# mwickert/scikit-dsp-comm

Measured on AMD Instinct MI355X. Metric: complex64 MSamples/s (FIR-1024 tap, 2^26 samples), higher is better.
Workload: dtype c64

## Files before the change

### scikit-dsp-comm_amd/csrc/fir_ols.hip

```cpp
#include "skdsp_internal.hpp"
#include "ols_tables.hpp"
#include "fir_route.hpp"
#include <cstdlib>
#include <cstdio>


namespace skdsp {

using namespace ols;
typedef float v4f_t __attribute__((ext_vector_type(4)));

struct OlsPlan : TilePlan {
    int ntaps = 0;
    int ov = 0;
    int V = 0;
    DevTable<float4> T1, T2, Hp;
};

struct OlsArgs {
    const cf *x;
    cf *y;
    int64_t n, n_hist;
    const float4 *T1, *T2, *Hp;
    int ov, V, a0;
    int keep;
    int aligned;
    int64_t ntiles;
    int dec;
    unsigned dec_magic;
    int up;
    int64_t up_pitch;
    int up_sb, up_pbs, up_pb0;
    int64_t n_keep;
    const unsigned *halo_flag;
    unsigned halo_seq;
    unsigned *halo_err;
    int halo_spins;
    CarefulFir cf;
    int rep_L, rep_lr;
    unsigned rep_magic;
    int64_t n_in, rep_hist;
};

__device__ __forceinline__ void wait_halo(const OlsArgs &A)
{
    if (threadIdx.x == 0) {
        int spins = 0;
        while ((int)(__hip_atomic_load(A.halo_flag, __ATOMIC_RELAXED, __HIP_MEMORY_SCOPE_AGENT) - A.halo_seq) < 0) {
            if (++spins > A.halo_spins) {
                *A.halo_err = 1u;
                break;
            }
            __builtin_amdgcn_s_sleep(16);
        }
        __builtin_amdgcn_fence(__ATOMIC_ACQUIRE, "agent");
    }
    __syncthreads();
}

static inline int ols_keep_blocks(int a0)
{
    const int o = opt().ols_keep_overlap;
    return o == 0 ? 0 : (o == 1 ? a0 : 8);
}

__device__ __forceinline__ float4 vld(const volatile float4 *p)
{
    float4 r;
    r.x = p->x; r.y = p->y; r.z = p->z; r.w = p->w;
    return r;
}

#define SK_GLOBAL_PTR(T, p) ((__attribute__((address_space(1))) T *)(p))
struct ScalarBase {
    uint64_t b;
    int g = 0;
    __device__ __forceinline__ explicit ScalarBase(const void *start) : b(reinterpret_cast<uint64_t>(start)) { asm volatile("" : "+s"(b)); }
    template <class T> __device__ __forceinline__ __attribute__((address_space(1))) T *at(int d, unsigned off)
    {
        const int gn = (d + 4096) >> 13;
        if (gn != g) {
            b += (uint64_t)(int64_t)(8192 * (gn - g));
            asm volatile("" : "+s"(b));
            g = gn;
        }
        return reinterpret_cast<__attribute__((address_space(1))) T *>(SK_GLOBAL_PTR(char, b) + off + (d - 8192 * gn));
    }
};

template <int KEEP, int A> __device__ __forceinline__ void load_tile_block(ScalarBase &xb, unsigned off, cf *v)
{
    const __attribute__((address_space(1))) v4f_t *src = xb.at<const v4f_t>(A * 4096, off);
    v4f_t nv;
    if constexpr (A < KEEP || A >= 16 - KEEP) nv = *src;
    else nv = __builtin_nontemporal_load(src);
    const float4 f = make_float4(nv.x, nv.y, nv.z, nv.w);
    v[2 * A] = lo(f);
    v[2 * A + 1] = hi(f);
    if constexpr (A < 15) load_tile_block<KEEP, A + 1>(xb, off, v);
}
template <int KEEP> __device__ __forceinline__ void load_tile_blocks(const cf *x0, int t, cf *v)
{
    int tt = t;
    asm volatile("" : "+v"(tt));
    ScalarBase xb(x0);
    load_tile_block<KEEP, 0>(xb, 16u * (unsigned)tt, v);
}

__device__ __forceinline__ void load_tile(const OlsArgs &A, int64_t tile, int t, cf *v)
{
    const int64_t in0 = tile * A.V - A.ov;
    const bool interior = A.aligned && in0 >= -A.n_hist && in0 + kN <= A.n;
    if (interior) {
        switch (A.keep) {
            case 0: load_tile_blocks<0>(A.x + in0, t, v); break;
            case 1: load_tile_blocks<1>(A.x + in0, t, v); break;
            case 2: load_tile_blocks<2>(A.x + in0, t, v); break;
            case 3: load_tile_blocks<3>(A.x + in0, t, v); break;
            case 4: load_tile_blocks<4>(A.x + in0, t, v); break;
            case 5: load_tile_blocks<5>(A.x + in0, t, v); break;
            case 6: load_tile_blocks<6>(A.x + in0, t, v); break;
            case 7: load_tile_blocks<7>(A.x + in0, t, v); break;
            default: load_tile_blocks<8>(A.x + in0, t, v); break;
        }
// ... 311 lines not shown
    const int64_t left = A.n - outA;
    const int lim = (left > (1 << 20) ? (1 << 20) : (int)left) - pos;
    const int limb = lim - A.V;
    const bool whole = left >= 2 * (int64_t)A.V;
    const unsigned b0 = (unsigned)pos * (unsigned)A.up_sb, b1 = b0 + 64u * (unsigned)A.up_sb;
    const size_t step = (size_t)512 * A.up_sb;
    const unsigned M = (unsigned)A.dec;
    const int64_t jt = outA * A.up + ph, q0 = DEC ? jt / A.dec : 0;
    const unsigned r0 = DEC ? (unsigned)(jt - q0 * A.dec) : 0u;
    const int64_t qleft = A.n_keep - q0;
    const int qlim = qleft > (1 << 24) ? (1 << 24) : (int)qleft;
    float *yq = reinterpret_cast<float *>(A.y) + q0;
    const unsigned jv = (unsigned)A.V * (unsigned)A.up;
#pragma unroll
    for (int a = 0; a < 16; ++a) {
        if (a < a0) continue;
        cf e0 = v[2 * a], e1 = v[2 * a + 1];
        lanes_swap_halves(e0.x, e1.x);
        lanes_swap_halves(e0.y, e1.y);
        const int i = 512 * (a - a0);
        if (DEC) {
            const unsigned j0 = r0 + (unsigned)(i + pos) * (unsigned)A.up, j1 = j0 + 64u * (unsigned)A.up;
            auto keep = [&](unsigned j, float val, bool inside) __attribute__((always_inline)) {
                const unsigned k = (unsigned)(((unsigned long long)j * A.dec_magic) >> 32);
                if (k * M == j && (int)k < qlim && inside) yq[k] = val;
            };
            keep(j0, e0.x, whole || i < lim);
            keep(j1, e1.x, whole || i + 64 < lim);
            keep(j0 + jv, e0.y, whole || i < limb);
            keep(j1 + jv, e1.y, whole || i + 64 < limb);
            continue;
        }
        char *ua = ua0 + (size_t)(a - a0) * step, *ub = ub0 + (size_t)(a - a0) * step;
        if (whole || i < lim) *reinterpret_cast<float *>(ua + b0) = e0.x;
        if (whole || i + 64 < lim) *reinterpret_cast<float *>(ua + b1) = e1.x;
        if (whole || i < limb) *reinterpret_cast<float *>(ub + b0) = e0.y;
        if (whole || i + 64 < limb) *reinterpret_cast<float *>(ub + b1) = e1.y;
    }
}


__device__ __forceinline__ OlsCareful ols_careful_args(const OlsArgs &A, int ph, bool cx)
{
    OlsCareful c;
    c.x = A.x; c.y = A.y; c.n = A.n; c.n_hist = A.n_hist; c.n_keep = A.n_keep; c.up_pitch = A.up_pitch;
    c.V = A.V; c.dec = A.dec; c.up = A.up;
    const int esz = cx ? 8 : 4;
    c.L = A.up_sb / esz;
    c.p0 = (A.up_pb0 + ph * A.up_pbs) / esz;
    c.cf = A.cf;
    return c;
}

template <bool REAL, bool DEC, bool UP = false, bool XR = false>
__global__ __launch_bounds__(256, 2) void ols_tile_kernel(OlsArgs A)
{
    __shared__ float4 lds[kLdsUnits];
    __shared__ float4 t2lds[2 * kT2Units];
    __shared__ unsigned long long ols_noted;
    if (threadIdx.x == 0) ols_noted = 0;
    constexpr int HS = (DEC && !UP) ? (REAL ? 4 : 5) : 0;
    float4 *T2f = t2lds;
    float4 *T2t = t2lds + kT2Units;
    const int t = threadIdx.x;

    {
        const float4 w = A.T2[t];
        T2f[t] = w;
        T2t[(t & 15) * 16 + (t >> 4)] = w;
    }
    cf tw[16];
#pragma unroll
    for (int k1 = 1; k1 < 16; ++k1) tw[k1] = lo(A.T1[k1 * 256 + t]);
    tw[0] = make_float2(1.f, 0.f);

    __syncthreads();
    int it = 0;
    float4 hh[16];
    int64_t tile = (gridDim.x % 8 == 0) ? (int64_t)(blockIdx.x % 8) * (gridDim.x / 8) + blockIdx.x / 8
                                                                 : (int64_t)blockIdx.x;
    const bool t0_last = A.halo_flag != nullptr;
    auto phys = [&](int64_t w) -> int64_t {
        if (UP) return (int64_t)__builtin_amdgcn_readfirstlane((unsigned)w / (unsigned)A.up);
        return t0_last ? (w + 1 < A.ntiles ? w + 1 : 0) : w;
    };
    auto phase_of = [&](int64_t w) -> int { return (int)__builtin_amdgcn_readfirstlane((unsigned)w % (unsigned)A.up); };
    if (!UP) load_H(t, A.Hp, hh);
    cf v[32];
    if (tile < A.ntiles) {
        if (t0_last && phys(tile) == 0) wait_halo(A);
        load_any<REAL, XR>(A, phys(tile), t, v);
    }
    if constexpr (XR) {
#pragma unroll
        for (int i = 0; i < 32; i += 8)
            asm volatile("" ::"v"(v[i].x), "v"(v[i + 1].x), "v"(v[i + 2].x), "v"(v[i + 3].x), "v"(v[i + 4].x), "v"(v[i + 5].x), "v"(v[i + 6].x), "v"(v[i + 7].x));
    } else {
#pragma unroll
    for (int i = 0; i < 32; i += 8)
        asm volatile("" ::"v"(v[i].x), "v"(v[i].y), "v"(v[i + 1].x), "v"(v[i + 1].y), "v"(v[i + 2].x), "v"(v[i + 2].y),
                     "v"(v[i + 3].x), "v"(v[i + 3].y), "v"(v[i + 4].x), "v"(v[i + 4].y), "v"(v[i + 5].x), "v"(v[i + 5].y),
                     "v"(v[i + 6].x), "v"(v[i + 6].y), "v"(v[i + 7].x), "v"(v[i + 7].y));
    }
    for (; tile < A.ntiles; tile += gridDim.x, ++it) {
        if (HS > 0) {
            int tt = t;
            asm volatile("" : "+v"(tt));
#pragma unroll
            for (int j = 16 - HS; j < 16; ++j) hh[j] = vld(reinterpret_cast<const volatile float4 *>(A.Hp) + (unsigned)(j * 256 + tt));
        }
        if (UP) {
            int tt = t;
            asm volatile("" : "+v"(tt));
            const volatile float4 *hp = reinterpret_cast<const volatile float4 *>(A.Hp) + (size_t)phase_of(tile) * 4096;
#pragma unroll
            for (int j = 0; j < 16; ++j) hh[j] = vld(hp + (unsigned)(j * 256 + tt));
        }
        if (REAL) fwd_pass1_real(t, v, tw, lds); else fwd_pass1(t, v, tw, lds);
        __syncthreads();
        cf Z[32];
        fwd_pass23(t, T2f, lds, Z);
        mul_H(hh, Z);
        const int64_t next = tile + gridDim.x;
        cf nx[32];
        __builtin_amdgcn_s_setprio(3);
        if (next < A.ntiles) {
            if (t0_last && phys(next) == 0) wait_halo(A);
            load_any<REAL, XR>(A, phys(next), t, nx);
        }
        __builtin_amdgcn_s_setprio(0);
        inv_pass32(t, T2t, lds, Z);
        __syncthreads();
        inv_pass1(t, tw, lds, v);
        if constexpr (XR) {
#pragma unroll
            for (int i = 0; i < 32; i += 8)
                asm volatile("" ::"v"(nx[i].x), "v"(nx[i + 1].x), "v"(nx[i + 2].x), "v"(nx[i + 3].x), "v"(nx[i + 4].x), "v"(nx[i + 5].x), "v"(nx[i + 6].x), "v"(nx[i + 7].x)
                             : "memory");
        } else {
#pragma unroll
        for (int i = 0; i < 32; i += 8)
            asm volatile("" ::"v"(nx[i].x), "v"(nx[i].y), "v"(nx[i + 1].x), "v"(nx[i + 1].y), "v"(nx[i + 2].x), "v"(nx[i + 2].y),
                         "v"(nx[i + 3].x), "v"(nx[i + 3].y), "v"(nx[i + 4].x), "v"(nx[i + 4].y), "v"(nx[i + 5].x), "v"(nx[i + 5].y),
                         "v"(nx[i + 6].x), "v"(nx[i + 6].y), "v"(nx[i + 7].x), "v"(nx[i + 7].y)
                         : "memory");
        }
        __builtin_amdgcn_s_setprio(3);
        if (UP) {
            if (!DEC && A.up_pitch) {
                OlsArgs B = A;
                B.y = REAL ? reinterpret_cast<cf *>(reinterpret_cast<float *>(A.y) + (int64_t)phase_of(tile) * A.up_pitch) : A.y + (int64_t)phase_of(tile) * A.up_pitch;
                store_any<REAL, false>(B, phys(tile), t, v, lds);
            } else if (REAL) {
                store_tile_real_up<DEC>(A, phys(tile), phase_of(tile), t, v);
            } else {
                store_tile_up<DEC>(A, phys(tile), phase_of(tile), t, v);
            }
        } else {
            store_any<REAL, DEC>(A, phys(tile), t, v, lds);
        }
        __builtin_amdgcn_s_setprio(0);
        if (__builtin_expect(__any(not_finite(v[31].x) | not_finite(v[31].y)), 0)) careful_note(&ols_noted, it);
#pragma unroll
        for (int i = 0; i < 32; ++i) v[i] = nx[i];
#ifdef SK_OLS_KEEP_B3
        __syncthreads();
#else
        if constexpr (REAL || DEC || UP || XR) __syncthreads();
#endif
    }
    const unsigned long long noted = careful_noted(&ols_noted);
    if (__builtin_expect(noted != 0, 0)) {
        int64_t w = (gridDim.x % 8 == 0) ? (int64_t)(blockIdx.x % 8) * (gridDim.x / 8) + blockIdx.x / 8 : (int64_t)blockIdx.x;
        for (int64_t k = 0; w < A.ntiles; w += gridDim.x, ++k)
            if (careful_step_noted(noted, k))
                careful_ols_tile<float, REAL, DEC, UP, XR>(ols_careful_args(A, UP ? phase_of(w) : 0, !(REAL || XR)), phys(w), UP ? phase_of(w) : 0, t);
    }
}


template <bool REAL, int MF>
__global__ __launch_bounds__(256, 2) void ols_fold_kernel(OlsArgs A)
{
    __shared__ float4 lds[kLdsUnits];
    __shared__ float4 t2lds[2 * kT2Units];
    __shared__ unsigned long long ols_noted;
    if (threadIdx.x == 0) ols_noted = 0;
    float4 *T2f = t2lds, *T2t = t2lds + kT2Units;
    const int t = threadIdx.x;
    {
        const float4 w = A.T2[t];
        T2f[t] = w;
        T2t[(t & 15) * 16 + (t >> 4)] = w;
    }
    cf tw[16];
#pragma unroll
    for (int k1 = 1; k1 < 16; ++k1) tw[k1] = lo(A.T1[k1 * 256 + t]);
    tw[0] = make_float2(1.f, 0.f);
    __syncthreads();
    float4 hh[16];
    auto first_tile = [&]() -> int64_t { return (gridDim.x % 8 == 0) ? (int64_t)(blockIdx.x % 8) * (gridDim.x / 8) + blockIdx.x / 8 : (int64_t)blockIdx.x; };
    int64_t tile = first_tile();
    load_H(t, A.Hp, hh);
    cf v[32];
    if (tile < A.ntiles) load_any<REAL, false>(A, tile, t, v);
#pragma unroll
    for (int i = 0; i < 32; i += 8)
        asm volatile("" ::"v"(v[i].x), "v"(v[i].y), "v"(v[i + 1].x), "v"(v[i + 1].y), "v"(v[i + 2].x), "v"(v[i + 2].y),
                     "v"(v[i + 3].x), "v"(v[i + 3].y), "v"(v[i + 4].x), "v"(v[i + 4].y), "v"(v[i + 5].x), "v"(v[i + 5].y),
                     "v"(v[i + 6].x), "v"(v[i + 6].y), "v"(v[i + 7].x), "v"(v[i + 7].y));
    constexpr int LS = MF / 2;
    const int b = t >> 4, q = t & 15;
    const bool active = q % LS == 0;
    const int j0 = (32 / MF) * b + q / LS;
    constexpr int JA = 512 / MF;
    for (int64_t step = 0; tile < A.ntiles; tile += gridDim.x, ++step) {
        if (REAL) fwd_pass1_real(t, v, tw, lds); else fwd_pass1(t, v, tw, lds);
        __syncthreads();
        cf Z[32];
        fwd_pass23(t, T2f, lds, Z);
        mul_H(hh, Z);
        const int64_t next = tile + gridDim.x;
        cf nx[32];
        __builtin_amdgcn_s_setprio(3);
        if (next < A.ntiles) load_any<REAL, false>(A, next, t, nx);
        __builtin_amdgcn_s_setprio(0);
        inv_pass32_fold<MF>(t, T2t, lds, Z);
        __syncthreads();
        cf o[16];
#pragma unroll
        for (int a = 0; a < 16; ++a) o[a] = make_float2(0.f, 0.f);
        inv_pass1_fold<MF>(t, tw, lds, o);
#pragma unroll
        for (int i = 0; i < 32; i += 8)
            asm volatile("" ::"v"(nx[i].x), "v"(nx[i].y), "v"(nx[i + 1].x), "v"(nx[i + 1].y), "v"(nx[i + 2].x), "v"(nx[i + 2].y),
                         "v"(nx[i + 3].x), "v"(nx[i + 3].y), "v"(nx[i + 4].x), "v"(nx[i + 4].y), "v"(nx[i + 5].x), "v"(nx[i + 5].y),
                         "v"(nx[i + 6].x), "v"(nx[i + 6].y), "v"(nx[i + 7].x), "v"(nx[i + 7].y)
                         : "memory");
        __builtin_amdgcn_s_setprio(3);
        if (active) {
            int a0 = A.a0;
            asm volatile("" : "+s"(a0));
            const int Mr = A.dec / MF;
            const int64_t n_out = A.n_keep / A.dec;
            const int VD = A.V / MF;
            const int64_t e0 = (REAL ? 2 * tile : tile) * (int64_t)VD;
            const int64_t q0 = Mr > 1 ? e0 / Mr : e0;
            const unsigned r0 = Mr > 1 ? (unsigned)(e0 - q0 * Mr) : 0u;
            auto put = [&](unsigned el, auto val, auto *yp) __attribute__((always_inline)) {
                if (Mr > 1) {
// ... 65 lines not shown
    int tt = j0;
    asm volatile("" : "+v"(tt));
    if (interior) {
        asm volatile("" : "+v"(tt));
        if (REAL) {
            const float *xr = reinterpret_cast<const float *>(A.x) + e0;
            const unsigned off = 4u * (unsigned)tt;
            ScalarBase xa(xr), xb(xr + VD);
#pragma unroll
            for (int a = 0; a < 16; ++a)
                in[a] = make_float2(__builtin_nontemporal_load(xa.at<const float>(JA * 4 * a, off)), __builtin_nontemporal_load(xb.at<const float>(JA * 4 * a, off)));
        } else {
            const unsigned off = 8u * (unsigned)tt;
            ScalarBase xc(A.x + e0);
#pragma unroll
            for (int a = 0; a < 16; ++a) {
                const v2f_t r = __builtin_nontemporal_load(xc.at<const v2f_t>(JA * 8 * a, off));
                in[a] = make_float2(r.x, r.y);
            }
        }
        return;
    }
#pragma unroll
    for (int a = 0; a < 16; ++a) {
        int64_t ia, ib;
        if (REAL) {
            const float *xr = reinterpret_cast<const float *>(A.x);
            float va = 0.f, vb = 0.f;
            if (fetch((unsigned)(JA * a + tt), ia) && ia >= -A.rep_hist && ia < A.n_in) va = xr[ia];
            if (fetch((unsigned)(JA * a + tt + VD), ib) && ib >= -A.rep_hist && ib < A.n_in) vb = xr[ib];
            in[a] = make_float2(va, vb);
        } else if (fetch((unsigned)(JA * a + tt), ia) && ia >= -A.rep_hist && ia < A.n_in) {
            in[a] = A.x[ia];
        }
    }
}

template <bool REAL, int LF>
__global__ __launch_bounds__(256, 2) void ols_rep_kernel(OlsArgs A)
{
    __shared__ float4 lds[kLdsUnits];
    __shared__ float4 t2lds[2 * kT2Units];
    __shared__ unsigned long long ols_noted;
    if (threadIdx.x == 0) ols_noted = 0;
    float4 *T2f = t2lds, *T2t = t2lds + kT2Units;
    const int t = threadIdx.x;
    {
        const float4 w = A.T2[t];
        T2f[t] = w;
        T2t[(t & 15) * 16 + (t >> 4)] = w;
    }
    cf tw[16];
#pragma unroll
    for (int k1 = 1; k1 < 16; ++k1) tw[k1] = lo(A.T1[k1 * 256 + t]);
    tw[0] = make_float2(1.f, 0.f);
    __syncthreads();
    float4 hh[16];
    auto first_tile = [&]() -> int64_t { return (gridDim.x % 8 == 0) ? (int64_t)(blockIdx.x % 8) * (gridDim.x / 8) + blockIdx.x / 8 : (int64_t)blockIdx.x; };
    int64_t tile = first_tile();
    load_H(t, A.Hp, hh);
    cf in[16];
    if (tile < A.ntiles) load_rep<REAL, LF>(A, tile, t, in);
#pragma unroll
    for (int i = 0; i < 16; i += 8)
        asm volatile("" ::"v"(in[i].x), "v"(in[i].y), "v"(in[i + 1].x), "v"(in[i + 1].y), "v"(in[i + 2].x), "v"(in[i + 2].y),
                     "v"(in[i + 3].x), "v"(in[i + 3].y), "v"(in[i + 4].x), "v"(in[i + 4].y), "v"(in[i + 5].x), "v"(in[i + 5].y),
                     "v"(in[i + 6].x), "v"(in[i + 6].y), "v"(in[i + 7].x), "v"(in[i + 7].y));
    for (int64_t step = 0; tile < A.ntiles; tile += gridDim.x, ++step) {
        fwd_pass1_rep<LF>(t, in, tw, lds);
        __syncthreads();
        cf Z[32];
        fwd_pass23_rep<LF>(t, T2f, lds, Z);
        mul_H(hh, Z);
        const int64_t next = tile + gridDim.x;
        cf nx[16];
        __builtin_amdgcn_s_setprio(3);
        if (next < A.ntiles) load_rep<REAL, LF>(A, next, t, nx);
        __builtin_amdgcn_s_setprio(0);
        inv_pass32(t, T2t, lds, Z);
        __syncthreads();
        cf v[32];
        inv_pass1(t, tw, lds, v);
#pragma unroll
        for (int i = 0; i < 16; i += 8)
            asm volatile("" ::"v"(nx[i].x), "v"(nx[i].y), "v"(nx[i + 1].x), "v"(nx[i + 1].y), "v"(nx[i + 2].x), "v"(nx[i + 2].y),
                         "v"(nx[i + 3].x), "v"(nx[i + 3].y), "v"(nx[i + 4].x), "v"(nx[i + 4].y), "v"(nx[i + 5].x), "v"(nx[i + 5].y),
                         "v"(nx[i + 6].x), "v"(nx[i + 6].y), "v"(nx[i + 7].x), "v"(nx[i + 7].y)
                         : "memory");
        __builtin_amdgcn_s_setprio(3);
        store_any<REAL, false>(A, tile, t, v, lds);
        __builtin_amdgcn_s_setprio(0);
        if (__builtin_expect(__any(not_finite(v[31].x) | not_finite(v[31].y)), 0)) careful_note(&ols_noted, step);
#pragma unroll
        for (int i = 0; i < 16; ++i) in[i] = nx[i];
        __syncthreads();
    }
    const unsigned long long noted = careful_noted(&ols_noted);
    if (__builtin_expect(noted != 0, 0)) {
        int64_t w = first_tile();
        for (int64_t k = 0; w < A.ntiles; w += gridDim.x, ++k)
            if (careful_step_noted(noted, k))
                careful_fir_range<float, !REAL>(A.x, A.y, A.rep_hist, A.n, (REAL ? 2 * w : w) * (int64_t)A.V, (REAL ? 2 : 1) * (int64_t)A.V, A.rep_L, 1, A.cf, t);
    }
}

static int build_plan(const FirHandle *h, int up, OlsPlan *p, int kind)
{
// ... 19 lines not shown
            make_Hp(ph.data(), T, 2, Hp);
            Hall.insert(Hall.end(), Hp.begin(), Hp.end());
        }
    } else if (up == 1) {
        make_Hp(h->taps_host.data(), h->ntaps, comp, Hall);
    } else if (kind == 3) {
        std::vector<double> scaled(h->taps_host);
        for (double &v : scaled) v *= (double)up;
        make_Hp(scaled.data(), h->ntaps, comp, Hall);
    } else {
        std::vector<double> ph((size_t)T * comp);
        for (int q = q_first; q < up; ++q) {
            std::fill(ph.begin(), ph.end(), 0.0);
            for (int t = 0; t < T; ++t) {
                const int k = q + up * t;
                if (k >= h->ntaps) break;
                for (int c = 0; c < comp; ++c) ph[(size_t)t * comp + c] = (double)up * h->taps_host[(size_t)k * comp + c];
            }
            make_Hp(ph.data(), T, comp, Hp);
            Hall.insert(Hall.end(), Hp.begin(), Hp.end());
        }
    }
    int rc;
    if ((rc = p->T1.upload(T1)) || (rc = p->T2.upload(T2)) || (rc = p->Hp.upload(Hall))) return rc;
    return SKDSP_OK;
}

static int ols_plan(FirHandle *h, int L, int kind, OlsPlan **out)
{
    return tile_plan(h->ols, plan_key(kind, L), out, [&](OlsPlan &p) { return build_plan(h, L, &p, kind); });
}

int fir_ols_tile_outputs(FirHandle *h, int *V)
{
    OlsPlan *p = nullptr;
    int rc = ols_plan(h, 1, 0, &p);
    if (rc) return rc;
    *V = p->V;
    return SKDSP_OK;
}

__global__ void ols_halo_flag_kernel(unsigned *flag, unsigned seq)
{
    __builtin_amdgcn_fence(__ATOMIC_RELEASE, "agent");
    __hip_atomic_store(flag, seq, __ATOMIC_RELAXED, __HIP_MEMORY_SCOPE_AGENT);
}

int fir_ols_publish_halo(unsigned *flag, unsigned seq, hipStream_t s)
{
    hipLaunchKernelGGL(ols_halo_flag_kernel, dim3(1), dim3(1), 0, s, flag, seq);
    SK_HIP(hipGetLastError());
    return SKDSP_OK;
}

int fir_ols_launch(FirHandle *h, const void *x, int64_t n, int64_t n_hist, void *y, hipStream_t s, int dec, int reserve_wgs,
                   const unsigned *halo_flag, unsigned halo_seq, unsigned *halo_err, int halo_spins)
{
    note_path("fir_ols");
    if (n <= 0) return SKDSP_OK;
    if (dec > 1) n = (n / dec) * dec;
    if (n <= 0) return SKDSP_OK;
    SK_CHECK(fir_ols_supported(fir_shape_of(h)), SKDSP_ERR_UNSUPPORTED, "fir_ols: needs complex64 (or float32 with real taps) and 2..4097 taps");
    SK_CHECK(dec <= 32768, SKDSP_ERR_UNSUPPORTED, "fir_ols: decimation by %d (the decimating store takes M <= 32768)", dec);
    OlsPlan *p = nullptr;
    int rc = ols_plan(h, 1, 0, &p);
    if (rc) return rc;
    OlsArgs A;
    A.x = (const cf *)x;
    A.y = (cf *)y;
    A.n = n;
    A.n_hist = n_hist;
    A.T1 = p->T1.dev; A.T2 = p->T2.dev; A.Hp = p->Hp.dev;
    A.ov = p->ov; A.V = p->V; A.a0 = p->ov / 512; A.keep = ols_keep_blocks(A.a0);
    const bool real = h->dtype == SKDSP_F32;
    A.aligned = ((((uintptr_t)x) | ((uintptr_t)y)) & (real ? 3 : 7)) == 0;
    int64_t ntiles = (n + p->V - 1) / p->V;
    if (real) ntiles = (ntiles + 1) / 2;
    SK_CHECK(ntiles < (int64_t)1 << 31, SKDSP_ERR_BADARG, "fir_ols: too many tiles");
    A.ntiles = ntiles;
    A.dec = dec > 1 ? dec : 1;
    A.dec_magic = A.dec > 1 ? (unsigned)((((unsigned long long)1 << 32) + A.dec - 1) / A.dec) : 0u;
    A.n_keep = n;
    A.up = 1; A.up_pitch = 0; A.up_sb = A.up_pbs = A.up_pb0 = 0;
    A.halo_flag = halo_flag; A.halo_seq = halo_seq; A.halo_err = halo_err; A.halo_spins = halo_spins > 0 ? halo_spins : (1 << 21);
    A.rep_L = 0; A.rep_lr = 1; A.rep_magic = 0; A.n_in = 0; A.rep_hist = 0;
    if ((rc = fir_careful(h, &A.cf))) return rc;
    SK_CHECK(!(halo_flag && real), SKDSP_ERR_UNSUPPORTED, "fir_ols: halo flag wait is for complex64 shards");
    int64_t grid = 2 * (int64_t)ctx().num_cus;
    if (reserve_wgs < 0) reserve_wgs = opt().ols_reserve;
    if (reserve_wgs > 0 && grid >= 4 * (int64_t)reserve_wgs) grid -= reserve_wgs;
    if (grid > ntiles) grid = ntiles;
    const int mf = A.dec % 16 == 0 ? 16 : (A.dec % 8 == 0 ? 8 : (A.dec % 4 == 0 ? 4 : (A.dec % 2 == 0 ? 2 : 1)));
    const bool fold = opt().fir_dn_fold && !halo_flag && mf > 1;
    if (fold) {
        const int mr = A.dec / mf;
        A.dec_magic = mr > 1 ? (unsigned)((((unsigned long long)1 << 32) + mr - 1) / mr) : 0u;
#define SK_FOLD(MF)                                                                                                  \
    if (real) hipLaunchKernelGGL((ols_fold_kernel<true, MF>), dim3((unsigned)grid), dim3(256), 0, s, A);             \
    else hipLaunchKernelGGL((ols_fold_kernel<false, MF>), dim3((unsigned)grid), dim3(256), 0, s, A)
        switch (mf) {
        case 2: SK_FOLD(2); break;
        case 4: SK_FOLD(4); break;
        case 8: SK_FOLD(8); break;
        default: SK_FOLD(16); break;
        }
#undef SK_FOLD
    } else if (A.dec > 1) {
        if (real) hipLaunchKernelGGL((ols_tile_kernel<true, true>), dim3((unsigned)grid), dim3(256), 0, s, A);
        else hipLaunchKernelGGL((ols_tile_kernel<false, true>), dim3((unsigned)grid), dim3(256), 0, s, A);
    } else {
        if (real) hipLaunchKernelGGL((ols_tile_kernel<true, false>), dim3((unsigned)grid), dim3(256), 0, s, A);
        else hipLaunchKernelGGL((ols_tile_kernel<false, false>), dim3((unsigned)grid), dim3(256), 0, s, A);
    }
    SK_HIP(hipGetLastError());
    return SKDSP_OK;
}


static int up_walk(FirHandle *h, int kind, const void *x, int64_t n, int64_t n_hist, int L, void *y, hipStream_t s, int dec, int64_t rows_pitch)
{
    OlsPlan *p = nullptr;
    int rc = ols_plan(h, L, kind, &p);
    if (rc) return rc;
    const bool xr = kind == 1;
    const bool real = h->dtype == SKDSP_F32 && !xr;
    const int cnt = kind == 1 ? L / 2 : (kind == 2 ? 1 : L);
    OlsArgs A;
    A.x = (const cf *)x;
    A.y = (cf *)y;
    A.n = n;
    A.n_hist = n_hist;
    A.T1 = p->T1.dev; A.T2 = p->T2.dev; A.Hp = p->Hp.dev;
    A.ov = p->ov; A.V = p->V; A.a0 = p->ov / 512; A.keep = ols_keep_blocks(A.a0);
    const int esz = h->dtype == SKDSP_F32 ? 4 : 8;
    A.aligned = xr ? (((uintptr_t)x & 3) == 0 && ((uintptr_t)y & (L % 2 ? 3 : 7)) == 0) : ((((uintptr_t)x) | ((uintptr_t)y)) & (real ? 3 : 7)) == 0;
    int64_t ntiles = (n + p->V - 1) / p->V;
    if (real) ntiles = (ntiles + 1) / 2;
    ntiles *= cnt;
    SK_CHECK(ntiles < (int64_t)1 << 31, SKDSP_ERR_BADARG, "fir_ols_up: too many tiles");
    A.ntiles = ntiles;
    A.dec = dec;
    A.dec_magic = dec > 1 ? (unsigned)((((unsigned long long)1 << 32) + dec - 1) / dec) : 0u;
    A.n_keep = dec > 1 ? (n * L) / dec : n;
    A.up = cnt;
    A.up_pitch = dec > 1 ? 0 : rows_pitch;
    A.up_sb = L * esz;
    A.up_pbs = xr ? 8 : esz;
    A.up_pb0 = kind == 2 ? (L - 1) * esz : 0;
    A.halo_flag = nullptr; A.halo_seq = 0; A.halo_err = nullptr; A.halo_spins = 0;
    A.rep_L = 0; A.rep_lr = 1; A.rep_magic = 0; A.n_in = 0; A.rep_hist = 0;
    if ((rc = fir_careful(h, &A.cf))) return rc;
    int64_t grid = 2 * (int64_t)ctx().num_cus;
    const int reserve_wgs = opt().ols_reserve;
    if (reserve_wgs > 0 && grid >= 4 * (int64_t)reserve_wgs) grid -= reserve_wgs;
    if (grid > ntiles) grid = ntiles;
    if (xr) {
        if (L == 2 && A.up_pitch == 0) A.up_pitch = 1;
        hipLaunchKernelGGL((ols_tile_kernel<false, false, true, true>), dim3((unsigned)grid), dim3(256), 0, s, A);
    } else if (dec > 1) {
        if (real) hipLaunchKernelGGL((ols_tile_kernel<true, true, true>), dim3((unsigned)grid), dim3(256), 0, s, A);
        else hipLaunchKernelGGL((ols_tile_kernel<false, true, true>), dim3((unsigned)grid), dim3(256), 0, s, A);
    } else {
        if (real) hipLaunchKernelGGL((ols_tile_kernel<true, false, true>), dim3((unsigned)grid), dim3(256), 0, s, A);
        else hipLaunchKernelGGL((ols_tile_kernel<false, false, true>), dim3((unsigned)grid), dim3(256), 0, s, A);
    }
    SK_HIP(hipGetLastError());
    return SKDSP_OK;
}

int fir_ols_rep_launch(FirHandle *h, const void *x, int64_t n, int64_t n_hist, int L, void *y, hipStream_t s)
{
    note_path("fir_ols_rep");
    if (n <= 0) return SKDSP_OK;
    SK_CHECK(fir_ols_rep_supported(fir_shape_of(h), L, opt().fir_up_rep), SKDSP_ERR_UNSUPPORTED, "fir_ols_rep: needs complex64 (or float32 with real taps), an even L and 2..4097 taps");
    OlsPlan *p = nullptr;
    int rc = ols_plan(h, L, 3, &p);
    if (rc) return rc;
    const bool real = h->dtype == SKDSP_F32;
    const int lf = L % 16 == 0 ? 16 : (L % 8 == 0 ? 8 : (L % 4 == 0 ? 4 : 2));
    OlsArgs A;
    A.x = (const cf *)x;
    A.y = (cf *)y;
    A.n = n * L;
    A.n_hist = n_hist * L;
    A.T1 = p->T1.dev; A.T2 = p->T2.dev; A.Hp = p->Hp.dev;
    A.ov = p->ov; A.V = p->V; A.a0 = p->ov / 512; A.keep = ols_keep_blocks(A.a0);
    A.aligned = ((((uintptr_t)x) | ((uintptr_t)y)) & (real ? 3 : 7)) == 0;
    int64_t ntiles = (A.n + p->V - 1) / p->V;
    if (real) ntiles = (ntiles + 1) / 2;
    SK_CHECK(ntiles < (int64_t)1 << 31, SKDSP_ERR_BADARG, "fir_ols_rep: too many tiles");
    A.ntiles = ntiles;
    A.dec = 1; A.dec_magic = 0; A.n_keep = A.n;
    A.up = 1; A.up_pitch = 0; A.up_sb = A.up_pbs = A.up_pb0 = 0;
    A.halo_flag = nullptr; A.halo_seq = 0; A.halo_err = nullptr; A.halo_spins = 0;
    A.rep_L = L; A.rep_lr = L / lf;
    A.rep_magic = A.rep_lr > 1 ? (unsigned)((((unsigned long long)1 << 32) + A.rep_lr - 1) / A.rep_lr) : 0u;
    A.n_in = n; A.rep_hist = n_hist;
    if ((rc = fir_careful(h, &A.cf))) return rc;
    int64_t grid = 2 * (int64_t)ctx().num_cus;
    const int reserve_wgs = opt().ols_reserve;
    if (reserve_wgs > 0 && grid >= 4 * (int64_t)reserve_wgs) grid -= reserve_wgs;
    if (grid > ntiles) grid = ntiles;
#define SK_REP(LFV)                                                                                                  \
    if (real) hipLaunchKernelGGL((ols_rep_kernel<true, LFV>), dim3((unsigned)grid), dim3(256), 0, s, A);             \
    else hipLaunchKernelGGL((ols_rep_kernel<false, LFV>), dim3((unsigned)grid), dim3(256), 0, s, A)
    switch (lf) {
    case 2: SK_REP(2); break;
    case 4: SK_REP(4); break;
    case 8: SK_REP(8); break;
    default: SK_REP(16); break;
    }
#undef SK_REP
    SK_HIP(hipGetLastError());
    return SKDSP_OK;
}

int fir_ols_up_launch(FirHandle *h, const void *x, int64_t n, int64_t n_hist, int L, void *y, hipStream_t s, int dec, int64_t rows_pitch, int paired)
{
    note_path("fir_ols_up");
    if (n <= 0) return SKDSP_OK;
    SK_CHECK(dec >= 1 && dec <= 4096 && (dec == 1 || L <= 64), SKDSP_ERR_UNSUPPORTED, "fir_ols_up: L / M = %d / %d (the fused L / M store takes L <= 64, M <= 4096)", L, dec);
    SK_CHECK(fir_ols_up_supported(fir_shape_of(h), L), SKDSP_ERR_UNSUPPORTED, "fir_ols_up: needs complex64 (or float32 with real taps), 2 <= L <= 256, 2..4097 taps per phase");
    if (!paired) return up_walk(h, 0, x, n, n_hist, L, y, s, dec, rows_pitch);
    SK_CHECK(fir_ols_up_pairs(fir_shape_of(h), L, dec, (unsigned)(uintptr_t)y, opt().fir_up_pair) && (L % 2 == 0 || rows_pitch == 0), SKDSP_ERR_BADARG,
             "fir_ols_up: phases in pairs need float32, real taps, no decimation, and an 8-byte aligned destination (even L) or the strided form (odd L, 7 .. 13)");
    int rc = up_walk(h, 1, x, n, n_hist, L, y, s, 1, rows_pitch);
    if (rc || L % 2 == 0) return rc;
    return up_walk(h, 2, x, n, n_hist, L, y, s, 1, 0);
}

}
```

### scikit-dsp-comm_amd/csrc/runtime.hip

```cpp
#include "api_internal.hpp"
#include <cstdarg>
#include <cstdio>
#include <cstdlib>
#include <cstring>

namespace skdsp {

static thread_local char g_err[1024] = "";

void set_error(const char *fmt, ...)
{
    va_list ap;
    va_start(ap, fmt);
    vsnprintf(g_err, sizeof(g_err), fmt, ap);
    va_end(ap);
}

int hip_fail(hipError_t e, const char *what, const char *file, int line)
{
    set_error("HIP error %d (%s) in %s at %s:%d", (int)e, hipGetErrorString(e), what, file, line);
    (void)hipGetLastError();
    if (e == hipErrorOutOfMemory) return SKDSP_ERR_NOMEM;
    if (e == hipErrorNoDevice || e == hipErrorInvalidDevice) return SKDSP_ERR_NODEVICE;
    return SKDSP_ERR_HIP;
// ... 31 lines not shown
    SK_HIP(hipSetDevice(g_slots[slot].device));
    return SKDSP_OK;
}

unsigned *async_err_dev(int which)
{
    Context &c = ctx();
    if (!c.async_err) {
        if (hipHostMalloc((void **)&c.async_err, kAsyncErrWords * sizeof(unsigned), hipHostMallocMapped) != hipSuccess) {
            (void)hipGetLastError();
            c.async_err = nullptr;
            return nullptr;
        }
        for (int i = 0; i < kAsyncErrWords; ++i) c.async_err[i] = 0;
    }
    unsigned *dev = nullptr;
    if (hipHostGetDevicePointer((void **)&dev, c.async_err, 0) != hipSuccess) return nullptr;
    return dev + which;
}

int async_err_check(Context &c)
{
    if (!c.async_err) return SKDSP_OK;
    volatile unsigned *w = c.async_err;
    if (w[kAsyncErrHalo]) {
        w[kAsyncErrHalo] = 0;
        opt().shard_two_launches = 1;
        set_error("fir_filter_shard: a sharded step since the last synchronisation gave up waiting for its halo inside the filter "
                  "launch (the first tile of that step is invalid); switched to the two-launch form (option shard_two_launches) -- "
                  "repeat the step on every rank");
        return SKDSP_ERR_RCCL;
    }
    if (w[kAsyncErrIirLookback]) {
        w[kAsyncErrIirLookback] = 0;
        set_error("iir: a look-back poll of a single-pass scan launched since the last synchronisation timed out (the results of "
                  "that call are invalid; option iir_two_pass = 1 selects the two-pass scan)");
        return SKDSP_ERR_HIP;
    }
    return SKDSP_OK;
}

int sync_checked()
{
    SK_HIP(hipStreamSynchronize(ctx().stream));
    return async_err_check(ctx());
}

namespace {
struct OptEntry { const char *name; int Options::*field; };
const OptEntry kOptTable[] = {
    {"device", &Options::device}, {"fir_algo", &Options::fir_algo}, {"dn_no_ols", &Options::dn_no_ols},
    {"fir_mm", &Options::fir_mm}, {"fir_bx", &Options::fir_bx}, 
    
    {"ols_reserve", &Options::ols_reserve}, {"fir_bx_t16", &Options::fir_bx_t16}, {"fir_bank_per", &Options::fir_bank_per}, {"ols_keep_overlap", &Options::ols_keep_overlap}, {"fir_dn_fold", &Options::fir_dn_fold}, {"fir_up_rep", &Options::fir_up_rep}, {"iir_seq", &Options::iir_seq}, {"psd_f32_image", &Options::psd_f32_image}, {"iir_up_jump", &Options::iir_up_jump}, {"iir_dn_t96", &Options::iir_dn_t96}, {"iir_up_lean", &Options::iir_up_lean}, {"iir_planar", &Options::iir_planar}, 
    {"iir_dn_full", &Options::iir_dn_full}, {"iir_no_mfma", &Options::iir_no_mfma}, 
    {"iir_two_pass", &Options::iir_two_pass}, {"iir_par", &Options::iir_par}, {"iir_par_v32", &Options::iir_par_v32}, {"iir_up_fused", &Options::iir_up_fused}, {"fir_up_ols_min", &Options::fir_up_ols_min}, {"fir_updn_fused", &Options::fir_updn_fused}, {"fir_up4k", &Options::fir_up4k}, {"fir_up4k_group", &Options::fir_up4k_group}, {"fir_up4k_staged", &Options::fir_up4k_staged}, {"fir_up2k", &Options::fir_up2k}, {"fir_dn4k", &Options::fir_dn4k}, {"fir_up_pair", &Options::fir_up_pair}, {"fir_up_rows_min", &Options::fir_up_rows_min}, {"iir_dn_compact", &Options::iir_dn_compact}, 
    {"shard_two_launches", &Options::shard_two_launches}, {"shard_probe", &Options::shard_probe}, {"shard_halo_state", &Options::shard_halo_state},
    {"shard_self_halo", &Options::shard_self_halo}, {"dist_force_comm", &Options::dist_force_comm},
    {"host_chunk_log2", &Options::host_chunk_log2}, {"host_pipeline", &Options::host_pipeline}, {"host_multi_slot", &Options::host_multi_slot}, {"pulse_mf_variant", &Options::pulse_mf_variant},
};
int parse_opt(const char *name, const char *v)
{
    if (!strcmp(name, "fir_algo")) {
        if (!strcmp(v, "direct")) return SKDSP_FIR_DIRECT;
        if (!strcmp(v, "ols")) return SKDSP_FIR_OLS;
        if (!strcmp(v, "auto")) return SKDSP_FIR_AUTO;
    }
    if (!*v) return 1;
    return atoi(v);
}
Options options_from_env()
{
    Options o;
    for (const OptEntry &e : kOptTable) {
        char key[64] = "SKDSP_";
        size_t k = 6;
        for (const char *p = e.name; *p && k + 1 < sizeof(key); ++p) key[k++] = (char)toupper((unsigned char)*p);
        key[k] = 0;
        if (const char *v = getenv(key)) o.*(e.field) = parse_opt(e.name, v);
    }
    return o;
}
}

Options &opt()
{
    static Options o = options_from_env();
    return o;
}

static int init_locked(int device)
{
    Context &c = ctx();
    if (c.ready) {
        SK_CHECK(device < 0 || device == c.device, SKDSP_ERR_BADARG,
                 "skdsp_init: slot %d is already bound to device %d", c.slot, c.device);
        return SKDSP_OK;
    }
    int ndev = 0;
    hipError_t e = hipGetDeviceCount(&ndev);
    if (e != hipSuccess || ndev <= 0) {
        set_error("no HIP device available (hipGetDeviceCount -> %d, %s): the MI355X path has no CPU fallback",
                  ndev, e == hipSuccess ? "0 devices" : hipGetErrorString(e));
        (void)hipGetLastError();
        return SKDSP_ERR_NODEVICE;
    }
    if (device < 0) device = 0;
// ... 293 lines not shown
```

### scikit-dsp-comm_amd/csrc/skdsp_internal.hpp

```cpp
#pragma once
#include <hip/hip_runtime.h>
#include <stdint.h>
#include <string>
#include <vector>
#include <memory>
#include <mutex>
#include "../../include/skdsp.h"
#include "careful.hpp"
#include "dev_mem.hpp"

namespace skdsp {

void set_error(const char *fmt, ...);
int hip_fail(hipError_t e, const char *what, const char *file, int line);

#define SK_HIP(call)                                                        \
    do {                                                                    \
        hipError_t _e = (call);                                             \
        if (_e != hipSuccess) return skdsp::hip_fail(_e, #call, __FILE__, __LINE__); \
    } while (0)

#define SK_CHECK(cond, code, ...)            \
    do {                                     \
        if (!(cond)) {                       \
            skdsp::set_error(__VA_ARGS__);   \
            return (code);                   \
        }                                    \
    } while (0)

void note_path(const char *engine);

struct Options {
    int device = -1;
    int fir_algo = 0;
    int dn_no_ols = 0;
    int fir_mm = 1;
    int fir_bx = 1;
    int fir_bx_t16 = 1;
    int ols_keep_overlap = 1;
    int ols_reserve = 8;
    int iir_planar = 0;
    int iir_dn_full = 0;
    int iir_no_mfma = 0;
    int iir_two_pass = 0;
    int iir_par = 1;
    int iir_par_v32 = 1;
    int iir_up_jump = 1;
    int iir_seq = 1;
    int iir_up_lean = 1;
    int iir_dn_t96 = 1;
    int iir_dn_compact = 1;
    int fir_up_ols_min = 64;
    int fir_up_rows_min = -1;
    int fir_up_pair = 1;
    int fir_up4k = 1;
    int fir_up2k = 1;
    int fir_up_rep = 1;
    int fir_dn_fold = 1;
    int fir_dn4k = 1;
    int fir_up4k_group = 4;
    int fir_up4k_staged = 1;
    int fir_bank_per = 0;
    int fir_updn_fused = 1;
    int iir_up_fused = 1;
    int shard_two_launches = 0;
    int shard_probe = 1;
    int shard_halo_state = 0;
    int shard_self_halo = 0;
    int dist_force_comm = 0;
    int host_chunk_log2 = 22;
    int host_pipeline = 1;
    int psd_f32_image = 0;
    int host_multi_slot = 1;
    int pulse_mf_variant = 0;
};
Options &opt();

constexpr int kMaxSlots = 16;
struct HostPipe;
struct Context {
    bool ready = false;
    int slot = 0;
    int device = -1;
    HostPipe *pipe = nullptr;
    int num_cus = 256;
    hipStream_t stream = nullptr;
    hipEvent_t ev_start = nullptr, ev_stop = nullptr;
    hipStream_t comm_stream = nullptr;
    hipEvent_t ev_in = nullptr, ev_halo = nullptr;
    unsigned *halo_flag = nullptr;
    unsigned *async_err = nullptr;
    unsigned halo_seq = 0;
    double last_timer_ms = -1.0;
// ... 223 lines not shown
```

Baseline: 299,600.

## Add atomic work-claiming tile walk with per-XCD ranges to OLS FIR kernel

Adds a dynamic tile scheduler to the OLS tile kernel. The tile range is split into eight ranges, each with its own atomic counter. Each workgroup claims tiles first from the range of its home XCD, then steals from the others, and it prefetches the next claim so the atomic overlaps with the load. The goal is to remove tail imbalance from the static grid-stride loop and keep each XCD on contiguous data. The cost is extra atomics, LDS for the tile history, a counter reset done by the last block, and more template instantiations. A compile-time timeline instrumentation path is also added.

```diff
diff --git a/scikit-dsp-comm_amd/csrc/fir_ols.hip b/scikit-dsp-comm_amd/csrc/fir_ols.hip
--- a/scikit-dsp-comm_amd/csrc/fir_ols.hip
+++ b/scikit-dsp-comm_amd/csrc/fir_ols.hip
@@ -1,6 +1,7 @@
 #include "skdsp_internal.hpp"
 #include "ols_tables.hpp"
 #include "fir_route.hpp"
+#include "ols_walk.hpp"
 #include <cstdlib>
 #include <cstdio>
 
@@ -15,6 +16,11 @@
     int ov = 0;
     int V = 0;
     DevTable<float4> T1, T2, Hp;
+    struct WalkCounters {
+        hipStream_t stream;
+        DevTable<unsigned> ctr;
+    };
+    std::vector<std::unique_ptr<WalkCounters>> walk;
 };
 
 struct OlsArgs {
@@ -40,7 +46,26 @@
     int rep_L, rep_lr;
     unsigned rep_magic;
     int64_t n_in, rep_hist;
+    unsigned *walk_ctr;
+#ifdef SKDSP_OLS_TIMELINE_BUILD
+    unsigned long long *tl;
+    int tl_steps;
+#endif
 };
+
+#ifdef SKDSP_OLS_TIMELINE_BUILD
+constexpr int kTlHead = 4;
+static unsigned long long *g_tl_buf = nullptr;
+static int g_tl_steps = 0;
+extern "C" void skdsp_ols_timeline_arm(void *buf_dev, int steps)
+{
+    g_tl_buf = (unsigned long long *)buf_dev;
+    g_tl_steps = steps;
+}
+#define SK_TL(...) do { __VA_ARGS__; } while (0)
+#else
+#define SK_TL(...) do { } while (0)
+#endif
 
 __device__ __forceinline__ void wait_halo(const OlsArgs &A)
 {
@@ -70,6 +95,8 @@
     r.x = p->x; r.y = p->y; r.z = p->z; r.w = p->w;
     return r;
 }
+
+__device__ __forceinline__ cf t1_lo(const float4 *T1, int i) { return *reinterpret_cast<const cf *>(T1 + i); }
 
 #define SK_GLOBAL_PTR(T, p) ((__attribute__((address_space(1))) T *)(p))
 struct ScalarBase {
@@ -487,12 +514,33 @@
     return c;
 }
 
-template <bool REAL, bool DEC, bool UP = false, bool XR = false>
+template <bool REAL, bool DEC, bool UP = false, bool XR = false, bool CLAIM = false>
 __global__ __launch_bounds__(256, 2) void ols_tile_kernel(OlsArgs A)
 {
     __shared__ float4 lds[kLdsUnits];
     __shared__ float4 t2lds[2 * kT2Units];
     __shared__ unsigned long long ols_noted;
+    __shared__ int walk_tiles[CLAIM ? olswalk::kMaxSteps : 1];
+    __shared__ unsigned walk_drawn;
+    __shared__ int walk_box[2];
+    olswalk::Walker wk = olswalk::walker((int)blockIdx.x);
+    unsigned drawn = 0;
+    bool in_flight = false;
+    auto draw_now = [&](olswalk::Walker u) {
+        int64_t idx = -1;
+        while (idx < 0 && !olswalk::walk_over(u)) idx = olswalk::take(u, A.ntiles, atomicAdd(A.walk_ctr + olswalk::draw_from(u), 1u));
+        walk_box[0] = (int)idx;
+        walk_box[1] = u.k;
+    };
+    auto read_box = [&]() -> int64_t {
+        const int idx = __builtin_amdgcn_readfirstlane(walk_box[0]);
+        wk.k = __builtin_amdgcn_readfirstlane(walk_box[1]);
+        if (idx < 0) return A.ntiles;
+        ++wk.steps;
+        return (int64_t)idx;
+    };
+    SK_TL(if (A.tl && threadIdx.x == 0) A.tl[(size_t)blockIdx.x * (kTlHead + 2 * A.tl_steps)] = wall_clock64());
+    if (CLAIM && threadIdx.x == 0) draw_now(wk);
     if (threadIdx.x == 0) ols_noted = 0;
     constexpr int HS = (DEC && !UP) ? (REAL ? 4 : 5) : 0;
     float4 *T2f = t2lds;
@@ -506,14 +554,16 @@
     }
     cf tw[16];
 #pragma unroll
-    for (int k1 = 1; k1 < 16; ++k1) tw[k1] = lo(A.T1[k1 * 256 + t]);
+    for (int k1 = 1; k1 < 16; ++k1) tw[k1] = t1_lo(A.T1, k1 * 256 + t);
     tw[0] = make_float2(1.f, 0.f);
 
     __syncthreads();
+    SK_TL(if (A.tl && threadIdx.x == 0) A.tl[(size_t)blockIdx.x * (kTlHead + 2 * A.tl_steps) + 1] = wall_clock64());
     int it = 0;
     float4 hh[16];
     int64_t tile = (gridDim.x % 8 == 0) ? (int64_t)(blockIdx.x % 8) * (gridDim.x / 8) + blockIdx.x / 8
                                                                  : (int64_t)blockIdx.x;
+    if constexpr (CLAIM) tile = read_box();
     const bool t0_last = A.halo_flag != nullptr;
     auto phys = [&](int64_t w) -> int64_t {
         if (UP) return (int64_t)__builtin_amdgcn_readfirstlane((unsigned)w / (unsigned)A.up);
@@ -525,6 +575,10 @@
     if (tile < A.ntiles) {
         if (t0_last && phys(tile) == 0) wait_halo(A);
         load_any<REAL, XR>(A, phys(tile), t, v);
+        if constexpr (CLAIM) {
+            in_flight = !olswalk::walk_over(wk);
+            if (in_flight && t == 0) drawn = atomicAdd(A.walk_ctr + olswalk::draw_from(wk), 1u);
+        }
     }
     if constexpr (XR) {
 #pragma unroll
@@ -537,7 +591,9 @@
                      "v"(v[i + 3].x), "v"(v[i + 3].y), "v"(v[i + 4].x), "v"(v[i + 4].y), "v"(v[i + 5].x), "v"(v[i + 5].y),
                      "v"(v[i + 6].x), "v"(v[i + 6].y), "v"(v[i + 7].x), "v"(v[i + 7].y));
     }
-    for (; tile < A.ntiles; tile += gridDim.x, ++it) {
+    if (CLAIM && in_flight && t == 0) walk_drawn = drawn;
+    for (; tile < A.ntiles; tile += CLAIM ? 0 : gridDim.x, ++it) {
+        if (CLAIM && t == 0) walk_tiles[it] = (int)tile;
         if (HS > 0) {
             int tt = t;
             asm volatile("" : "+v"(tt));
@@ -556,16 +612,32 @@
         cf Z[32];
         fwd_pass23(t, T2f, lds, Z);
         mul_H(hh, Z);
-        const int64_t next = tile + gridDim.x;
+        int64_t next = tile + gridDim.x;
+        if constexpr (CLAIM) {
+            next = A.ntiles;
+            if (in_flight) {
+                const int64_t idx = olswalk::take(wk, A.ntiles, (unsigned)__builtin_amdgcn_readfirstlane(walk_drawn));
+                if (idx >= 0) {
+                    next = idx;
+                } else if (!olswalk::walk_over(wk)) {
+                    if (t == 0) draw_now(wk);
+                    __syncthreads();
+                    next = read_box();
+                }
+            }
+            in_flight = next < A.ntiles && !olswalk::walk_over(wk);
+        }
         cf nx[32];
         __builtin_amdgcn_s_setprio(3);
         if (next < A.ntiles) {
             if (t0_last && phys(next) == 0) wait_halo(A);
+            if (CLAIM && in_flight && t == 0) drawn = atomicAdd(A.walk_ctr + olswalk::draw_from(wk), 1u);
             load_any<REAL, XR>(A, phys(next), t, nx);
         }
         __builtin_amdgcn_s_setprio(0);
         inv_pass32(t, T2t, lds, Z);
         __syncthreads();
+        if (CLAIM && in_flight && t == 0) walk_drawn = drawn;
         inv_pass1(t, tw, lds, v);
         if constexpr (XR) {
 #pragma unroll
@@ -595,7 +667,13 @@
             store_any<REAL, DEC>(A, phys(tile), t, v, lds);
         }
         __builtin_amdgcn_s_setprio(0);
+        SK_TL(if (A.tl && t == 0 && it < A.tl_steps) {
+            unsigned long long *rec = A.tl + (size_t)blockIdx.x * (kTlHead + 2 * A.tl_steps) + kTlHead + 2 * it;
+            rec[0] = wall_clock64();
+            rec[1] = (unsigned long long)phys(tile);
+        });
         if (__builtin_expect(__any(not_finite(v[31].x) | not_finite(v[31].y)), 0)) careful_note(&ols_noted, it);
+        if constexpr (CLAIM) tile = next;
 #pragma unroll
         for (int i = 0; i < 32; ++i) v[i] = nx[i];
 #ifdef SK_OLS_KEEP_B3
@@ -604,12 +682,29 @@
         if constexpr (REAL || DEC || UP || XR) __syncthreads();
 #endif
     }
+    if (CLAIM && t == 0) {
+        if (atomicAdd(A.walk_ctr + olswalk::kDone * olswalk::kCtrStride, 1u) == gridDim.x - 1)
+            for (int r = 0; r <= olswalk::kRanges; ++r) __hip_atomic_store(A.walk_ctr + r * olswalk::kCtrStride, 0u, __ATOMIC_RELAXED, __HIP_MEMORY_SCOPE_AGENT);
+    }
+    SK_TL(if (A.tl && t == 0) {
+        unsigned long long *rec = A.tl + (size_t)blockIdx.x * (kTlHead + 2 * A.tl_steps);
+        rec[2] = wall_clock64();
+        rec[3] = (unsigned long long)it;
+    });
     const unsigned long long noted = careful_noted(&ols_noted);
     if (__builtin_expect(noted != 0, 0)) {
         int64_t w = (gridDim.x % 8 == 0) ? (int64_t)(blockIdx.x % 8) * (gridDim.x / 8) + blockIdx.x / 8 : (int64_t)blockIdx.x;
+        if constexpr (CLAIM) {
+            for (int k = 0; k < it; ++k)
+                if (careful_step_noted(noted, k)) {
+                    w = __builtin_amdgcn_readfirstlane(walk_tiles[k]);
+                    careful_ols_tile<float, REAL, DEC, UP, XR>(ols_careful_args(A, UP ? phase_of(w) : 0, !(REAL || XR)), phys(w), UP ? phase_of(w) : 0, t);
+                }
+        } else {
         for (int64_t k = 0; w < A.ntiles; w += gridDim.x, ++k)
             if (careful_step_noted(noted, k))
                 careful_ols_tile<float, REAL, DEC, UP, XR>(ols_careful_args(A, UP ? phase_of(w) : 0, !(REAL || XR)), phys(w), UP ? phase_of(w) : 0, t);
+        }
     }
 }
 
@@ -630,7 +725,7 @@
     }
     cf tw[16];
 #pragma unroll
-    for (int k1 = 1; k1 < 16; ++k1) tw[k1] = lo(A.T1[k1 * 256 + t]);
+    for (int k1 = 1; k1 < 16; ++k1) tw[k1] = t1_lo(A.T1, k1 * 256 + t);
     tw[0] = make_float2(1.f, 0.f);
     __syncthreads();
     float4 hh[16];
@@ -802,7 +897,7 @@
     }
     cf tw[16];
 #pragma unroll
-    for (int k1 = 1; k1 < 16; ++k1) tw[k1] = lo(A.T1[k1 * 256 + t]);
+    for (int k1 = 1; k1 < 16; ++k1) tw[k1] = t1_lo(A.T1, k1 * 256 + t);
     tw[0] = make_float2(1.f, 0.f);
     __syncthreads();
     float4 hh[16];
@@ -928,6 +1023,28 @@
     SK_HIP(hipGetLastError());
     return SKDSP_OK;
 }
+
+static int walk_of_launch(OlsPlan *p, hipStream_t s, int64_t grid, bool plain, OlsArgs *A, bool *claim)
+{
+    A->walk_ctr = nullptr;
+    const int o = opt().ols_walk;
+    *claim = (o == 2 || (o == 1 && plain)) && olswalk::walk_takes(A->ntiles, grid);
+    if (!*claim) return SKDSP_OK;
+    for (auto &w : p->walk)
+        if (w->stream == s) { A->walk_ctr = w->ctr.dev; return SKDSP_OK; }
+    std::unique_ptr<OlsPlan::WalkCounters> w(new OlsPlan::WalkCounters());
+    w->stream = s;
+    const int rc = w->ctr.upload(std::vector<unsigned>(olswalk::kCtrWords, 0u));
+    if (rc) return rc;
+    A->walk_ctr = w->ctr.dev;
+    p->walk.push_back(std::move(w));
+    return SKDSP_OK;
+}
+#define SK_TILE(R, D, U, X)                                                                                           \
+    do {                                                                                                              \
+        if (claim) hipLaunchKernelGGL((ols_tile_kernel<R, D, U, X, true>), dim3((unsigned)grid), dim3(256), 0, s, A);  \
+        else hipLaunchKernelGGL((ols_tile_kernel<R, D, U, X>), dim3((unsigned)grid), dim3(256), 0, s, A);              \
+    } while (0)
 
 int fir_ols_launch(FirHandle *h, const void *x, int64_t n, int64_t n_hist, void *y, hipStream_t s, int dec, int reserve_wgs,
                    const unsigned *halo_flag, unsigned halo_seq, unsigned *halo_err, int halo_spins)
@@ -968,6 +1085,12 @@
     if (grid > ntiles) grid = ntiles;
     const int mf = A.dec % 16 == 0 ? 16 : (A.dec % 8 == 0 ? 8 : (A.dec % 4 == 0 ? 4 : (A.dec % 2 == 0 ? 2 : 1)));
     const bool fold = opt().fir_dn_fold && !halo_flag && mf > 1;
+    bool claim = false;
+    A.walk_ctr = nullptr;
+    if (!fold && (rc = walk_of_launch(p, s, grid, A.dec == 1 && !halo_flag, &A, &claim))) return rc;
+#ifdef SKDSP_OLS_TIMELINE_BUILD
+    A.tl = g_tl_buf; A.tl_steps = g_tl_steps;
+#endif
     if (fold) {
         const int mr = A.dec / mf;
         A.dec_magic = mr > 1 ? (unsigned)((((unsigned long long)1 << 32) + mr - 1) / mr) : 0u;
@@ -982,11 +1105,11 @@
         }
 #undef SK_FOLD
     } else if (A.dec > 1) {
-        if (real) hipLaunchKernelGGL((ols_tile_kernel<true, true>), dim3((unsigned)grid), dim3(256), 0, s, A);
-        else hipLaunchKernelGGL((ols_tile_kernel<false, true>), dim3((unsigned)grid), dim3(256), 0, s, A);
+        if (real) SK_TILE(true, true, false, false);
+        else SK_TILE(false, true, false, false);
     } else {
-        if (real) hipLaunchKernelGGL((ols_tile_kernel<true, false>), dim3((unsigned)grid), dim3(256), 0, s, A);
-        else hipLaunchKernelGGL((ols_tile_kernel<false, false>), dim3((unsigned)grid), dim3(256), 0, s, A);
+        if (real) SK_TILE(true, false, false, false);
+        else SK_TILE(false, false, false, false);
     }
     SK_HIP(hipGetLastError());
     return SKDSP_OK;
@@ -1030,15 +1153,20 @@
     const int reserve_wgs = opt().ols_reserve;
     if (reserve_wgs > 0 && grid >= 4 * (int64_t)reserve_wgs) grid -= reserve_wgs;
     if (grid > ntiles) grid = ntiles;
+    bool claim = false;
+    if ((rc = walk_of_launch(p, s, grid, false, &A, &claim))) return rc;
+#ifdef SKDSP_OLS_TIMELINE_BUILD
+    A.tl = nullptr; A.tl_steps = 0;
+#endif
     if (xr) {
         if (L == 2 && A.up_pitch == 0) A.up_pitch = 1;
-        hipLaunchKernelGGL((ols_tile_kernel<false, false, true, true>), dim3((unsigned)grid), dim3(256), 0, s, A);
+        SK_TILE(false, false, true, true);
     } else if (dec > 1) {
-        if (real) hipLaunchKernelGGL((ols_tile_kernel<true, true, true>), dim3((unsigned)grid), dim3(256), 0, s, A);
-        else hipLaunchKernelGGL((ols_tile_kernel<false, true, true>), dim3((unsigned)grid), dim3(256), 0, s, A);
+        if (real) SK_TILE(true, true, true, false);
+        else SK_TILE(false, true, true, false);
     } else {
-        if (real) hipLaunchKernelGGL((ols_tile_kernel<true, false, true>), dim3((unsigned)grid), dim3(256), 0, s, A);
-        else hipLaunchKernelGGL((ols_tile_kernel<false, false, true>), dim3((unsigned)grid), dim3(256), 0, s, A);
+        if (real) SK_TILE(true, false, true, false);
+        else SK_TILE(false, false, true, false);
     }
     SK_HIP(hipGetLastError());
     return SKDSP_OK;
@@ -1072,6 +1200,10 @@
     A.rep_L = L; A.rep_lr = L / lf;
     A.rep_magic = A.rep_lr > 1 ? (unsigned)((((unsigned long long)1 << 32) + A.rep_lr - 1) / A.rep_lr) : 0u;
     A.n_in = n; A.rep_hist = n_hist;
+    A.walk_ctr = nullptr;
+#ifdef SKDSP_OLS_TIMELINE_BUILD
+    A.tl = nullptr; A.tl_steps = 0;
+#endif
     if ((rc = fir_careful(h, &A.cf))) return rc;
     int64_t grid = 2 * (int64_t)ctx().num_cus;
     const int reserve_wgs = opt().ols_reserve;
diff --git a/scikit-dsp-comm_amd/csrc/ols_walk.hpp b/scikit-dsp-comm_amd/csrc/ols_walk.hpp
--- /dev/null
+++ b/scikit-dsp-comm_amd/csrc/ols_walk.hpp
@@ -0,0 +1,44 @@
+#pragma once
+#include <stdint.h>
+
+#if defined(__HIPCC__)
+#define SK_WALK_HD __host__ __device__ __forceinline__
+#else
+#define SK_WALK_HD inline
+#endif
+
+namespace skdsp {
+namespace olswalk {
+
+constexpr int kRanges = 8;
+constexpr int kMaxSteps = 896;
+constexpr int kCtrStride = 32;
+constexpr int kDone = kRanges;
+constexpr int kCtrWords = (kRanges + 1) * kCtrStride;
+
+SK_WALK_HD int64_t range_start(int64_t ntiles, int r) { return ntiles * r / kRanges; }
+SK_WALK_HD int range_of(int xcd, int k) { return (xcd + k) % kRanges; }
+SK_WALK_HD bool walk_takes(int64_t ntiles, int64_t grid) { return grid > 0 && ntiles <= grid * (int64_t)kMaxSteps; }
+
+struct Walker {
+    int xcd;
+    int k;
+    int steps;
+};
+SK_WALK_HD Walker walker(int block) { return Walker{block % kRanges, 0, 0}; }
+SK_WALK_HD bool walk_over(const Walker &w) { return w.k >= kRanges || w.steps >= kMaxSteps; }
+SK_WALK_HD int draw_from(const Walker &w) { return range_of(w.xcd, w.k) * kCtrStride; }
+SK_WALK_HD int64_t take(Walker &w, int64_t ntiles, unsigned drawn)
+{
+    const int r = range_of(w.xcd, w.k);
+    const int64_t s = range_start(ntiles, r), len = range_start(ntiles, r + 1) - s;
+    if ((int64_t)drawn < len) {
+        ++w.steps;
+        return s + (int64_t)drawn;
+    }
+    ++w.k;
+    return -1;
+}
+
+}
+}
diff --git a/scikit-dsp-comm_amd/csrc/runtime.hip b/scikit-dsp-comm_amd/csrc/runtime.hip
--- a/scikit-dsp-comm_amd/csrc/runtime.hip
+++ b/scikit-dsp-comm_amd/csrc/runtime.hip
@@ -107,7 +107,7 @@
     {"device", &Options::device}, {"fir_algo", &Options::fir_algo}, {"dn_no_ols", &Options::dn_no_ols},
     {"fir_mm", &Options::fir_mm}, {"fir_bx", &Options::fir_bx}, 
     
-    {"ols_reserve", &Options::ols_reserve}, {"fir_bx_t16", &Options::fir_bx_t16}, {"fir_bank_per", &Options::fir_bank_per}, {"ols_keep_overlap", &Options::ols_keep_overlap}, {"fir_dn_fold", &Options::fir_dn_fold}, {"fir_up_rep", &Options::fir_up_rep}, {"iir_seq", &Options::iir_seq}, {"psd_f32_image", &Options::psd_f32_image}, {"iir_up_jump", &Options::iir_up_jump}, {"iir_dn_t96", &Options::iir_dn_t96}, {"iir_up_lean", &Options::iir_up_lean}, {"iir_planar", &Options::iir_planar}, 
+    {"ols_reserve", &Options::ols_reserve}, {"ols_walk", &Options::ols_walk},{"fir_bx_t16", &Options::fir_bx_t16}, {"fir_bank_per", &Options::fir_bank_per}, {"ols_keep_overlap", &Options::ols_keep_overlap}, {"fir_dn_fold", &Options::fir_dn_fold}, {"fir_up_rep", &Options::fir_up_rep}, {"iir_seq", &Options::iir_seq}, {"psd_f32_image", &Options::psd_f32_image}, {"iir_up_jump", &Options::iir_up_jump}, {"iir_dn_t96", &Options::iir_dn_t96}, {"iir_up_lean", &Options::iir_up_lean}, {"iir_planar", &Options::iir_planar}, 
     {"iir_dn_full", &Options::iir_dn_full}, {"iir_no_mfma", &Options::iir_no_mfma}, 
     {"iir_two_pass", &Options::iir_two_pass}, {"iir_par", &Options::iir_par}, {"iir_par_v32", &Options::iir_par_v32}, {"iir_up_fused", &Options::iir_up_fused}, {"fir_up_ols_min", &Options::fir_up_ols_min}, {"fir_updn_fused", &Options::fir_updn_fused}, {"fir_up4k", &Options::fir_up4k}, {"fir_up4k_group", &Options::fir_up4k_group}, {"fir_up4k_staged", &Options::fir_up4k_staged}, {"fir_up2k", &Options::fir_up2k}, {"fir_dn4k", &Options::fir_dn4k}, {"fir_up_pair", &Options::fir_up_pair}, {"fir_up_rows_min", &Options::fir_up_rows_min}, {"iir_dn_compact", &Options::iir_dn_compact}, 
     {"shard_two_launches", &Options::shard_two_launches}, {"shard_probe", &Options::shard_probe}, {"shard_halo_state", &Options::shard_halo_state},
diff --git a/scikit-dsp-comm_amd/csrc/skdsp_internal.hpp b/scikit-dsp-comm_amd/csrc/skdsp_internal.hpp
--- a/scikit-dsp-comm_amd/csrc/skdsp_internal.hpp
+++ b/scikit-dsp-comm_amd/csrc/skdsp_internal.hpp
@@ -39,6 +39,7 @@
     int fir_bx_t16 = 1;
     int ols_keep_overlap = 1;
     int ols_reserve = 8;
+    int ols_walk = 1;
     int iir_planar = 0;
     int iir_dn_full = 0;
     int iir_no_mfma = 0;
```

Measured after the change: 311,000 (median of 6 runs). 3.8% higher.
